# Nyro-Robotics/booster_gym

Measured on AMD Instinct MI355X. Metric: env-steps/sec (whole node), PPO rollout+update, T1 4096 envs/GPU, higher is better.
Workload: dtype f32

## Files before the change

booster_gym_amd/csrc/bg_env.h:

```cpp
#pragma once
#include "../../include/booster_gym_amd.h"
#include "bg_dyn.h"
#include "bg_rng.h"

namespace bg {

enum {
    F_ROOT = 0,
    F_Q = 13,
    F_QD = 25,
    F_LAST_TGT = 37,
    F_ACT = 49,
    F_LAST_ACT = 61,
    F_LAST_QD = 73,
    F_LAST_ROOTVEL = 85,
    F_CMD = 91,
    F_GAIT_F = 94,
    F_GAIT_P = 95,
    F_FILT_LIN = 96,
    F_FILT_ANG = 99,
    F_LAST_FEET = 102,
    F_PUSH = 108,
    F_CONTACT = 114,
    F_KP = 120, F_KD = 132, F_FRIC = 144,
// ... 77 lines not shown
    if (K <= 1u) return 0u;
    uint32_t bits = 2u;
    while (bits < 32u && (1u << bits) < K) bits += 2u;
    const uint32_t hb = bits >> 1, hm = (1u << hb) - 1u;
    uint32_t x = p;
    for (int walk = 0; walk < 64; walk++) {
        uint32_t L = x >> hb, R = x & hm;
        for (uint32_t r = 0; r < 4u; r++) {
            const uint32_t f = mix32(R ^ (key + r * 0x9E3779B9u)) & hm;
            const uint32_t t = L ^ f;
            L = R; R = t;
        }
        x = (L << hb) | R;
        if (x < K) return x;
    }
    return p;
}

template <int I, class St>
BG_HD void leg_fk(const St& st, const LegParams& lp, const LegState& ls, M3 Rpar, V3 ppar, M3* Rf, V3* pf) {
    constexpr int AX = LEG_AXIS[I], J = Plane<AX>::J, K = Plane<AX>::K;
    float s, c;
    bg_sincos(ls.q[I], &s, &c);
    V3 p = ppar + mul(Rpar, st.template link_pos<I>(lp));
    M3 R = Rpar;
    for (int r = 0; r < 3; r++) {
        R.e[r][J] = c * Rpar.e[r][J] + s * Rpar.e[r][K];
        R.e[r][K] = -s * Rpar.e[r][J] + c * Rpar.e[r][K];
    }
    if constexpr (I + 1 < LEG_LINKS) leg_fk<I + 1>(st, lp, ls, R, p, Rf, pf);
    else { *Rf = R; *pf = p; }
}

BG_HD Phys make_phys(const bg_env_cfg& c) {
    Phys ph;
    ph.dt = c.sim_dt; ph.g = v3(c.gravity[0], c.gravity[1], c.gravity[2]);
    ph.contact_ramp = c.contact_ramp; ph.friction_visc = c.friction_visc; ph.limit_k = c.limit_k; ph.limit_d = c.limit_d; ph.clamp_qd = c.clamp_qd;
    ph.body_gate = c.body_gate_height; ph.body_kn = c.contact_k; ph.body_dn = c.contact_d * (1.0f - 0.5f * c.terrain_restitution);
    ph.body_mu = 0.5f * (1.0f + c.terrain_mu);
    ph.zmask = 0;
    ph.self_on = c.self_collisions; ph.self_k = c.self_k; ph.self_d = c.self_d; ph.self_mu = c.self_mu; ph.self_visc = c.self_visc;
    return ph;
}
BG_HD ContactCfg make_contact_cfg(const bg_env_cfg& c) {
    ContactCfg cc; cc.k = c.contact_k; cc.d = c.contact_d; cc.terrain_mu = c.terrain_mu; cc.terrain_restitution = c.terrain_restitution;
    return cc;
}

BG_HD float quat_yaw(const float q[4]) {
    float x = q[0], y = q[1], z = q[2], w = q[3];
    return atan2f(2.f * (w * z + x * y), w * w + x * x - y * y - z * z);
}

struct GlobalSink {
    static constexpr int SELF = SELF_INLINE;
    float* obs; float* priv; int e;
    BG_HD void put_obs(int k, float v) { obs[(size_t)e * BG_NUM_OBS + k] = v; }
    BG_HD void put_priv(int k, float v) { priv[(size_t)e * BG_NUM_PRIV + k] = v; }
};

template <bool H16>
struct FieldRef {
    float* pf;
    bg_half_bits* ph;
    BG_HD operator float() const {
        if constexpr (H16) { if (ph) return half_bits_to_float(*ph); }
        return *pf;
    }
    BG_HD void operator=(float v) const {
        if constexpr (H16) { if (ph) { *ph = float_to_half_bits(v); return; } }
        *pf = v;
    }
};
template <bool H16>
BG_HD FieldRef<H16> field_ref(float* F, bg_half_bits* H, int idx, int n, int e) {
    const size_t o = (size_t)idx * n + e;
    return FieldRef<H16>{F + o, (H16 && fp16_state_field(idx)) ? H + o : nullptr};
}

template <class X, class Sink, bool H16, bool BODY, bool TC = false>
BG_HD void env_step_lane(const EnvDev& E, X& x, Sink& sink, int e, int leg, bool valid, const float* act, uint32_t step, int mode,
                         const StepOut& out) {
    const bg_env_cfg& C = E.cfg;
    const int n = E.n;
    const ModelDev& M = *E.model;
    float* const F = E.f;
    bg_half_bits* const HS = E.h;
    int32_t* const II = E.i;
#define FLD(off, comp) field_ref<H16>(F, HS, (off) + (comp), n, e)
    const int j0 = leg * LEG_LINKS;
    const float dt_env = C.sim_dt * (float)C.decimation;
    Phys ph = make_phys(C);
    ph.zmask = E.zmask;
    ContactCfg cc = make_contact_cfg(C);

    BaseState bs;
    for (int a = 0; a < 3; a++) { bs.pos.e[a] = FLD(F_ROOT, a); bs.vlin.e[a] = FLD(F_ROOT, 7 + a); bs.vang.e[a] = FLD(F_ROOT, 10 + a); }
    for (int a = 0; a < 4; a++) bs.quat[a] = FLD(F_ROOT, 3 + a);
    LegState ls;
    float last_tgt[LEG_LINKS], kp[LEG_LINKS], kd[LEG_LINKS], fric[LEG_LINKS], a6[LEG_LINKS], last_act[LEG_LINKS], last_qd[LEG_LINKS];
    for (int i = 0; i < LEG_LINKS; i++) {
        ls.q[i] = FLD(F_Q, j0 + i); ls.qd[i] = FLD(F_QD, j0 + i);
        last_tgt[i] = FLD(F_LAST_TGT, j0 + i);
        kp[i] = FLD(F_KP, j0 + i); kd[i] = FLD(F_KD, j0 + i); fric[i] = FLD(F_FRIC, j0 + i);
        last_act[i] = FLD(F_LAST_ACT, j0 + i); last_qd[i] = FLD(F_LAST_QD, j0 + i);
    }
    LegParams lp;
    load_leg_params(M, cc, leg, e, n, F + (size_t)F_MASS_SCALE * n, F + (size_t)F_COM_OFF * n, F + (size_t)F_FOOT_MAT * n, lp);
    LinkConst bk = load_base_link(M, e, n, F + (size_t)F_MASS_SCALE * n, F + (size_t)F_COM_OFF * n);
    int ep_len = II[(size_t)I_EP_LEN * n + e], cmd_time = II[(size_t)I_CMD_TIME * n + e], delay = II[(size_t)I_DELAY * n + e];
    float cmd[3] = {FLD(F_CMD, 0), FLD(F_CMD, 1), FLD(F_CMD, 2)};
    float gait_f = FLD(F_GAIT_F, 0), gait_p = FLD(F_GAIT_P, 0);
    V3 filt_lin = v3(FLD(F_FILT_LIN, 0), FLD(F_FILT_LIN, 1), FLD(F_FILT_LIN, 2));
    V3 filt_ang = v3(FLD(F_FILT_ANG, 0), FLD(F_FILT_ANG, 1), FLD(F_FILT_ANG, 2));
    V3 push_f = v3(FLD(F_PUSH, 0), FLD(F_PUSH, 1), FLD(F_PUSH, 2)), push_t = v3(FLD(F_PUSH, 3), FLD(F_PUSH, 4), FLD(F_PUSH, 5));
    V3 last_foot = v3(FLD(F_LAST_FEET, 3 * leg), FLD(F_LAST_FEET, 3 * leg + 1), FLD(F_LAST_FEET, 3 * leg + 2));
    float last_rootvel[6];
    for (int a = 0; a < 6; a++) last_rootvel[a] = FLD(F_LAST_ROOTVEL, a);

    float tmean[LEG_LINKS];
    float body_pen = 0.f, body_term = 0.f;
    V3 foot_force = v3(0.f, 0.f, 0.f);
    for (int i = 0; i < LEG_LINKS; i++) { tmean[i] = 0.f; a6[i] = FLD(F_ACT, j0 + i); }

    typename Sink::Ctx cx;
    sink.bind(cx, lp);
    if (mode == 0) {
        float target[LEG_LINKS];
        for (int i = 0; i < LEG_LINKS; i++) {
            float a = act[(size_t)e * BG_NUM_DOFS + j0 + i];
            if (((float_bits(a) >> 23) & 0xFFu) == 0xFFu) a = 0.f;
            a = fminf(fmaxf(a, -C.clip_actions), C.clip_actions);
            a6[i] = a;
            target[i] = C.default_dof_pos[j0 + i] + C.action_scale * a;
        }
        SV wrench = local_wrench_at_com(bk, push_f, push_t);
        for (int s = 0; s < C.decimation; s++) {
            float tau[LEG_LINKS];
            for (int i = 0; i < LEG_LINKS; i++) {
                if (delay == s) last_tgt[i] = target[i];
                tau[i] = pd_torque(kp[i], kd[i], fric[i], M.tau_lim[j0 + i], last_tgt[i], ls.q[i], ls.qd[i]);
                tmean[i] += tau[i];
            }
            BodyContactOut bo;
            BaseContribution mine = substep_pre<BODY, Sink::SELF>(ph, E.terrain, M, leg, lp, ls, tau, bs, cx, x, (const SV*)nullptr, &bo);
            body_pen = 0.f; body_term = 0.f;
            if constexpr (BODY) {
                V3 tf = bo.trunk;
                for (int a = 0; a < 3; a++) tf.e[a] += x.swap(tf.e[a]);
                const float trunk_hit = (leg == 0 && dot(tf, tf) > 1.0f) ? 1.f : 0.f;
                body_pen = (C.penalized_body_mask & 1) ? trunk_hit : 0.f;
                body_term = (C.terminate_body_mask & 1) ? trunk_hit : 0.f;
                for (int i = 0; i < LEG_LINKS - 1; i++) {
                    const float hit = dot(bo.link[i], bo.link[i]) > 1.0f ? 1.f : 0.f;
                    const int bit = 1 << (1 + j0 + i);
                    if (C.penalized_body_mask & bit) body_pen += hit;
                    if (C.terminate_body_mask & bit) body_term += hit;
                }
            } else {
                const float hit = dot(bo.link[SELF_SHANK], bo.link[SELF_SHANK]) > 1.0f ? 1.f : 0.f;
                const int bit = 1 << (1 + j0 + SELF_SHANK);
                body_pen = (C.penalized_body_mask & bit) ? hit : 0.f;
                body_term = (C.terminate_body_mask & bit) ? hit : 0.f;
            }
            BaseContribution both;
            for (int k = 0; k < 6; k++) { both.I.A.e[k] = mine.I.A.e[k] + x.swap(mine.I.A.e[k]); both.I.M.e[k] = mine.I.M.e[k] + x.swap(mine.I.M.e[k]); }
            for (int r = 0; r < 3; r++) for (int c2 = 0; c2 < 3; c2++) both.I.H.e[r][c2] = mine.I.H.e[r][c2] + x.swap(mine.I.H.e[r][c2]);
            for (int k = 0; k < 3; k++) { both.p.a.e[k] = mine.p.a.e[k] + x.swap(mine.p.a.e[k]); both.p.l.e[k] = mine.p.l.e[k] + x.swap(mine.p.l.e[k]); }
            float qdd[LEG_LINKS];
            V3 lin_w, ang_w;
            SV wr = wrench;
            if (s != 0) wr = sv_zero();
            substep_solve(ph, bk, lp, ls, cx, both, wr, qdd, &lin_w, &ang_w, &foot_force);
            substep_integrate(ph, lp, ls, bs, qdd, lin_w, ang_w);
        }
        for (int i = 0; i < LEG_LINKS; i++) tmean[i] *= 1.0f / (float)C.decimation;
    }

    uint32_t expo = 0;
    {
        const float st[13] = {bs.pos.e[0], bs.pos.e[1], bs.pos.e[2], bs.quat[0], bs.quat[1], bs.quat[2], bs.quat[3],
                              bs.vlin.e[0], bs.vlin.e[1], bs.vlin.e[2], bs.vang.e[0], bs.vang.e[1], bs.vang.e[2]};
        for (int k = 0; k < 13; k++) expo |= (uint32_t)(((float_bits(st[k]) >> 23) & 0xFFu) >= 0xE6u);
        for (int i = 0; i < LEG_LINKS; i++) {
            expo |= (uint32_t)(((float_bits(ls.q[i]) >> 23) & 0xFFu) >= 0xE6u);
            expo |= (uint32_t)(((float_bits(ls.qd[i]) >> 23) & 0xFFu) >= 0xE6u);
        }
    }
    float bad = expo ? 1.f : 0.f;
    bad = (bad != 0.f || x.swap(bad) != 0.f) ? 1.f : 0.f;
    if (bad != 0.f) {
        bs.pos = v3(0.f, 0.f, 1.f); bs.quat[0] = bs.quat[1] = bs.quat[2] = 0.f; bs.quat[3] = 1.f;
        bs.vlin = v3(0.f, 0.f, 0.f); bs.vang = v3(0.f, 0.f, 0.f);
        for (int i = 0; i < LEG_LINKS; i++) { ls.q[i] = 0.f; ls.qd[i] = 0.f; tmean[i] = 0.f; }
        foot_force = v3(0.f, 0.f, 0.f);
    }
    M3 R0 = quat_to_mat(bs.quat);
    V3 base_lin = mulT(R0, bs.vlin), base_ang = mulT(R0, bs.vang);
    V3 proj_g = mulT(R0, v3(0.f, 0.f, -1.f));
    if (mode == 0) {
        filt_lin = C.filter_weight * base_lin + (1.0f - C.filter_weight) * filt_lin;
        filt_ang = C.filter_weight * base_ang + (1.0f - C.filter_weight) * filt_ang;
    }
    M3 Rf; V3 pf;
    leg_fk<0>(cx.w.st, lp, ls, R0, bs.pos, &Rf, &pf);
    float roll = atan2f(Rf.e[2][1], Rf.e[2][2]), yaw = atan2f(Rf.e[1][0], Rf.e[0][0]);
    float fcontact = 0.f;
    for (int k = 0; k < 4; k++) {
        V3 xw = pf + mul(Rf, lp.corner[k]);
        if (xw.e[2] - terrain_height(E.terrain, xw.e[0], xw.e[1]) < 0.01f) fcontact = 1.f;
    }
    float s_tau2 = 0.f, s_tired = 0.f, s_power = 0.f, s_qd2 = 0.f, s_acc = 0.f, s_arate = 0.f, s_poslim = 0.f, s_vellim = 0.f, s_taulim = 0.f;
    for (int i = 0; i < LEG_LINKS; i++) {
        float lim = M.tau_lim[j0 + i], lo = M.q_lo[j0 + i], hi = M.q_hi[j0 + i];
        s_tau2 += tmean[i] * tmean[i];
        float tr = tmean[i] / lim;
        s_tired += fminf(tr * tr, 1.0f);
        s_power += fmaxf(tmean[i] * ls.qd[i], 0.f);
        s_qd2 += ls.qd[i] * ls.qd[i];
        float acc = (last_qd[i] - ls.qd[i]) / dt_env;
        s_acc += acc * acc;
        float da = last_act[i] - a6[i];
        s_arate += da * da;
        float lower = lo + 0.5f * (1.f - C.soft_dof_pos_limit) * (hi - lo), upper = hi - 0.5f * (1.f - C.soft_dof_pos_limit) * (hi - lo);
        s_poslim += (ls.q[i] < lower || ls.q[i] > upper) ? 1.f : 0.f;
        s_vellim += fminf(fmaxf(fabsf(ls.qd[i]) - M.qd_max[j0 + i] * C.soft_dof_vel_limit, 0.f), 1.f);
        s_taulim += fmaxf(fabsf(tmean[i]) - lim * C.soft_torque_limit, 0.f);
    }
    V3 dfoot = (1.0f / dt_env) * (last_foot - pf);
    float slip_own = dot(dfoot, dfoot) * fcontact;
    float velz_own = dfoot.e[2] * dfoot.e[2];
    V3 pf_o = v3(x.swap(pf.e[0]), x.swap(pf.e[1]), x.swap(pf.e[2]));
    float roll_o = x.swap(roll), yaw_o = x.swap(yaw), fcontact_o = x.swap(fcontact);
    s_tau2 += x.swap(s_tau2); s_tired += x.swap(s_tired); s_power += x.swap(s_power); s_qd2 += x.swap(s_qd2); s_acc += x.swap(s_acc);
    s_arate += x.swap(s_arate); s_poslim += x.swap(s_poslim); s_vellim += x.swap(s_vellim); s_taulim += x.swap(s_taulim);
    float slip = slip_own + x.swap(slip_own), velz = velz_own + x.swap(velz_own);
    V3 foot_force_o = v3(x.swap(foot_force.e[0]), x.swap(foot_force.e[1]), x.swap(foot_force.e[2]));
    V3 pL = leg == 0 ? pf : pf_o, pR = leg == 0 ? pf_o : pf;
    float yawL = leg == 0 ? yaw : yaw_o, yawR = leg == 0 ? yaw_o : yaw, rollL = leg == 0 ? roll : roll_o, rollR = leg == 0 ? roll_o : roll;
    float conL = leg == 0 ? fcontact : fcontact_o, conR = leg == 0 ? fcontact_o : fcontact;

    uint8_t reset_flag = 0, tout_flag = 0;
    float rew_total = 0.f;
    float term[BG_NUM_REWARD_TERMS];
    for (int k = 0; k < BG_NUM_REWARD_TERMS; k++) term[k] = 0.f;
    const uint32_t cnt = step + 1;
    const uint32_t so = mode ? 64u : 0u;

    if (mode == 0) {
        ep_len += 1;
        gait_p = fmodf(gait_p + dt_env * gait_f, 1.0f);
        if (C.kick_interval > 0 && cnt % (uint32_t)C.kick_interval == 0) {
            Rand4 r0 = rand4(C.seed, (uint32_t)e, step, so + RS_KICK0), r1 = rand4(C.seed, (uint32_t)e, step, so + RS_KICK1);
            for (int a = 0; a < 3; a++) bs.vlin.e[a] = apply_rand(bs.vlin.e[a], C.kick_lin_vel, r0.u[a], r0.n[a]);
            bs.vang.e[0] = apply_rand(bs.vang.e[0], C.kick_ang_vel, r0.u[3], r0.n[3]);
            bs.vang.e[1] = apply_rand(bs.vang.e[1], C.kick_ang_vel, r1.u[0], r1.n[0]);
            bs.vang.e[2] = apply_rand(bs.vang.e[2], C.kick_ang_vel, r1.u[1], r1.n[1]);
        }
        if (C.push_interval > 0) {
            uint32_t ph_ = cnt % (uint32_t)C.push_interval;
            if (ph_ == 0) {
                Rand4 r0 = rand4(C.seed, (uint32_t)e, step, so + RS_PUSH0), r1 = rand4(C.seed, (uint32_t)e, step, so + RS_PUSH1);
                for (int a = 0; a < 3; a++) push_f.e[a] = apply_rand(0.f, C.push_force, r0.u[a], r0.n[a]);
                push_t.e[0] = apply_rand(0.f, C.push_torque, r0.u[3], r0.n[3]);
                push_t.e[1] = apply_rand(0.f, C.push_torque, r1.u[0], r1.n[0]);
                push_t.e[2] = apply_rand(0.f, C.push_torque, r1.u[1], r1.n[1]);
            } else if (ph_ == (uint32_t)C.push_duration) {
                push_f = v3(0.f, 0.f, 0.f); push_t = v3(0.f, 0.f, 0.f);
            }
        }
        float h_base = terrain_height(E.terrain, bs.pos.e[0], bs.pos.e[1]);
        float v2 = dot(bs.vlin, bs.vlin) + dot(bs.vang, bs.vang);
        bool to = ep_len > C.max_episode_length;
        {
            const float hit = dot(foot_force, foot_force) > 1.0f ? 1.f : 0.f;
            const int bit = 1 << (1 + j0 + LEG_LINKS - 1);
            if (C.penalized_body_mask & bit) body_pen += hit;
            if (C.terminate_body_mask & bit) body_term += hit;
        }
        body_pen += x.swap(body_pen);
        body_term += x.swap(body_term);
        bool rs = (body_term > 0.f) || (v2 > C.terminate_vel) || (bs.pos.e[2] - h_base < C.terminate_height) || to;
        to = to || (ep_len == cmd_time);
        if (bad != 0.f) rs = true;
        reset_flag = rs ? 1 : 0; tout_flag = to ? 1 : 0;
        float base_yaw = quat_yaw(bs.quat);
        float bh = bs.pos.e[2] - h_base - C.base_height_target;
        float ex = cmd[0] - filt_lin.e[0], ey = cmd[1] - filt_lin.e[1], ew = cmd[2] - filt_ang.e[2];
        float racc = 0.f;
        {
            float rv[6] = {bs.vlin.e[0], bs.vlin.e[1], bs.vlin.e[2], bs.vang.e[0], bs.vang.e[1], bs.vang.e[2]};
            for (int a = 0; a < 6; a++) { float d = (last_rootvel[a] - rv[a]) / dt_env; racc += d * d; }
        }
        float ydiff = wrap_pi(yawR - yawL);
        float ymean = 0.5f * (yawL + yawR) + (fabsf(yawR - yawL) > 3.14159265358979f ? 3.14159265358979f : 0.f);
        float ymerr = wrap_pi(base_yaw - ymean);
        float fdist = fabsf(cosf(base_yaw) * (pR.e[1] - pL.e[1]) - sinf(base_yaw) * (pR.e[0] - pL.e[0]));
        bool gait_on = gait_f > 1.0e-8f;
        bool lsw = (fabsf(gait_p - 0.25f) < 0.5f * C.swing_period) && gait_on, rsw = (fabsf(gait_p - 0.75f) < 0.5f * C.swing_period) && gait_on;
        term[BG_REW_SURVIVAL] = 1.0f;
        term[BG_REW_TRACKING_LIN_VEL_X] = expf(-ex * ex / C.tracking_sigma);
        term[BG_REW_TRACKING_LIN_VEL_Y] = expf(-ey * ey / C.tracking_sigma);
        term[BG_REW_TRACKING_ANG_VEL] = expf(-ew * ew / C.tracking_sigma);
        term[BG_REW_BASE_HEIGHT] = bh * bh;
        term[BG_REW_ORIENTATION] = proj_g.e[0] * proj_g.e[0] + proj_g.e[1] * proj_g.e[1];
        term[BG_REW_TORQUES] = s_tau2;
        term[BG_REW_TORQUE_TIREDNESS] = s_tired;
        term[BG_REW_POWER] = s_power;
        term[BG_REW_LIN_VEL_Z] = filt_lin.e[2] * filt_lin.e[2];
        term[BG_REW_ANG_VEL_XY] = base_ang.e[0] * base_ang.e[0] + base_ang.e[1] * base_ang.e[1];
        term[BG_REW_DOF_VEL] = s_qd2;
        term[BG_REW_DOF_ACC] = s_acc;
        term[BG_REW_ROOT_ACC] = racc;
        term[BG_REW_ACTION_RATE] = s_arate;
        term[BG_REW_DOF_POS_LIMITS] = s_poslim;
        term[BG_REW_DOF_VEL_LIMITS] = s_vellim;
        term[BG_REW_TORQUE_LIMITS] = s_taulim;
        term[BG_REW_COLLISION] = body_pen;
        term[BG_REW_FEET_SLIP] = slip * (ep_len > 1 ? 1.f : 0.f);
        term[BG_REW_FEET_VEL_Z] = velz;
        term[BG_REW_FEET_YAW_DIFF] = ydiff * ydiff;
        term[BG_REW_FEET_YAW_MEAN] = ymerr * ymerr;
        term[BG_REW_FEET_ROLL] = rollL * rollL + rollR * rollR;
        term[BG_REW_FEET_DISTANCE] = fminf(fmaxf(C.feet_distance_ref - fdist, 0.f), 0.1f);
        term[BG_REW_FEET_SWING] = ((lsw && conL == 0.f) ? 1.f : 0.f) + ((rsw && conR == 0.f) ? 1.f : 0.f);
        for (int k = 0; k < BG_NUM_REWARD_TERMS; k++) {
            term[k] = C.reward_scale[k] != 0.f ? term[k] * C.reward_scale[k] : 0.f;
            rew_total += term[k];
        }
        if (C.only_positive_rewards) rew_total = fmaxf(rew_total, 0.f);
        if (bad != 0.f) { rew_total = 0.f; for (int k = 0; k < BG_NUM_REWARD_TERMS; k++) term[k] = 0.f; }
    } else {
        reset_flag = 1;
    }

    V3 pf_store = pf;
    if (reset_flag && mode == 0 && C.curriculum && leg == 0 && valid && bad == 0.f) {
        const int nx = 2 * C.lin_vel_levels + 1, ny = 2 * C.ang_vel_levels + 1;
        bool success = (float)ep_len > ceilf((float)C.max_episode_length) * (1.0f - C.episode_length_toler);
        success = success && fabsf(filt_lin.e[0] - cmd[0]) < C.lin_vel_x_toler && fabsf(filt_lin.e[1] - cmd[1]) < C.lin_vel_y_toler &&
                  fabsf(filt_ang.e[2] - cmd[2]) < C.ang_vel_yaw_toler;
        if (success) {
            const int cx = II[(size_t)I_CURR_LIN * n + e] + C.lin_vel_levels, cy = II[(size_t)I_CURR_ANG * n + e] + C.ang_vel_levels;
            const float r = C.curriculum_update_rate;
#if defined(__HIP_DEVICE_COMPILE__)
#define BG_ACC(ix, iy) atomicAdd(&E.curr[(ix) * ny + (iy)], r)
#else
#define BG_ACC(ix, iy) (E.curr[(ix) * ny + (iy)] += r)
#endif
            BG_ACC(cx, cy);
            if (cx > 0) BG_ACC(cx - 1, cy);
            if (cx < nx - 1) BG_ACC(cx + 1, cy);
            if (cy > 0) BG_ACC(cx, cy - 1);
            if (cy < ny - 1) BG_ACC(cx, cy + 1);
#undef BG_ACC
        }
    }
    float org_x = 0.f, org_y = 0.f;
    if constexpr (TC) {
        org_x = FLD(F_ORIGIN, 0); org_y = FLD(F_ORIGIN, 1);
        if (reset_flag && mode == 0 && valid && bad == 0.f) {
            int32_t* const TL = E.tcur;
            const int lvl = TL[e], col = TL[(size_t)n + e];
            const float dx = bs.pos.e[0] - org_x, dy = bs.pos.e[1] - org_y;
            const float d = sqrtf(dx * dx + dy * dy);
            const bool up = d > 0.5f * C.terrain_tile_length;
            const bool down = !up && d < sqrtf(cmd[0] * cmd[0] + cmd[1] * cmd[1]) * C.terrain_down_time;
            int nl = lvl + (up ? 1 : 0) - (down ? 1 : 0);
            nl = nl < 0 ? 0 : nl;
            if (nl >= C.terrain_num_levels) {
                nl = (int)(rand4(C.seed, (uint32_t)e, step, RS_TLEVEL).u[0] * (float)C.terrain_num_levels);
                nl = nl < C.terrain_num_levels ? nl : C.terrain_num_levels - 1;
            }
            org_x = ((float)col + 0.5f) * C.terrain_tile_width;
            org_y = ((float)nl + 0.5f) * C.terrain_tile_length;
            if (leg == 0) {
                TL[e] = nl;
                FLD(F_ORIGIN, 0) = org_x; FLD(F_ORIGIN, 1) = org_y; FLD(F_ORIGIN, 2) = terrain_height(E.terrain, org_x, org_y);
                if (nl != lvl) {
#if defined(__HIP_DEVICE_COMPILE__)
                    atomicAdd(&TL[2 * (size_t)n], nl - lvl);
#else
                    TL[2 * (size_t)n] += nl - lvl;
#endif
                }
            }
        }
    }
    if (reset_flag) {
        uint32_t noise_env = C.shared_reset_noise ? 0xFFFFFFFFu : (uint32_t)e;
        Rand4 d0 = rand4(C.seed, noise_env, step, so + RS_RESETDOF + leg * 2), d1 = rand4(C.seed, noise_env, step, so + RS_RESETDOF + leg * 2 + 1);
        for (int i = 0; i < LEG_LINKS; i++) {
            float u = i < 4 ? d0.u[i] : d1.u[i - 4], nn = i < 4 ? d0.n[i] : d1.n[i - 4];
            ls.q[i] = apply_rand(C.default_dof_pos[j0 + i], C.init_dof_pos, u, nn);
            ls.qd[i] = 0.f;
            last_tgt[i] = ls.q[i];
        }
        Rand4 r0 = rand4(C.seed, (uint32_t)e, step, so + RS_RESET0), r1 = rand4(C.seed, (uint32_t)e, step, so + RS_RESET1);
        float px = apply_rand(C.base_init_state[0] + (TC ? org_x : (float)FLD(F_ORIGIN, 0)), C.init_base_pos_xy, r0.u[0], r0.n[0]);
        float py = apply_rand(C.base_init_state[1] + (TC ? org_y : (float)FLD(F_ORIGIN, 1)), C.init_base_pos_xy, r0.u[1], r0.n[1]);
        bs.pos = v3(px, py, C.base_init_state[2] + terrain_height(E.terrain, px, py));
        float yw = r0.u[2] * 6.28318530717959f, sy, cy;
        bg_sincos(0.5f * yw, &sy, &cy);
        bs.quat[0] = 0.f; bs.quat[1] = 0.f; bs.quat[2] = sy; bs.quat[3] = cy;
        bs.vlin = v3(apply_rand(0.f, C.init_base_lin_vel_xy, r1.u[0], r1.n[0]), apply_rand(0.f, C.init_base_lin_vel_xy, r1.u[1], r1.n[1]), C.base_init_state[9]);
        bs.vang = v3(C.base_init_state[10], C.base_init_state[11], C.base_init_state[12]);
        ep_len = 0; cmd_time = 0;
        filt_lin = v3(0.f, 0.f, 0.f); filt_ang = v3(0.f, 0.f, 0.f);
        int dl = (int)(r0.u[3] * (float)C.decimation);
        delay = dl < C.decimation ? dl : C.decimation - 1;
    }
    if (mode == 0 && C.terrain_type != 0) {
        float sx = 0.f, sy2 = 0.f;
        float wx = C.terrain_env_width + C.terrain_border, wy = C.terrain_env_length + C.terrain_border;
        if (bs.pos.e[0] < -0.75f * C.terrain_border) sx += wx;
        if (bs.pos.e[0] > C.terrain_env_width + 0.75f * C.terrain_border) sx -= wx;
        if (bs.pos.e[1] < -0.75f * C.terrain_border) sy2 += wy;
        if (bs.pos.e[1] > C.terrain_env_length + 0.75f * C.terrain_border) sy2 -= wy;
        bs.pos.e[0] += sx; bs.pos.e[1] += sy2;
        pf_store.e[0] += sx; pf_store.e[1] += sy2;
    }
    const bool defer_still = C.exact_still_count != 0, defer_curr = C.curriculum && C.same_step_curriculum != 0;
    int resampled = 0;
    if (ep_len == cmd_time) {
        resampled = 1;
        Rand4 c0 = rand4(C.seed, (uint32_t)e, step, so + RS_CMD0), c1 = rand4(C.seed, (uint32_t)e, step, so + RS_CMD1);
        if (C.curriculum && !defer_curr) {
            Rand4 cr = rand4(C.seed, (uint32_t)e, step, so + RS_CURR);
            int lin_level, ang_level;
            curriculum_draw(C, E.curr_read, cr, cmd, &lin_level, &ang_level);
            if (leg == 0 && valid) { II[(size_t)I_CURR_LIN * n + e] = lin_level; II[(size_t)I_CURR_ANG * n + e] = ang_level; }
        } else if (!C.curriculum) {
            cmd[0] = C.cmd_lin_vel_x[0] + (C.cmd_lin_vel_x[1] - C.cmd_lin_vel_x[0]) * c0.u[0];
            cmd[1] = C.cmd_lin_vel_y[0] + (C.cmd_lin_vel_y[1] - C.cmd_lin_vel_y[0]) * c0.u[1];
            cmd[2] = C.cmd_ang_vel_yaw[0] + (C.cmd_ang_vel_yaw[1] - C.cmd_ang_vel_yaw[0]) * c0.u[2];
        }
        gait_f = C.cmd_gait_frequency[0] + (C.cmd_gait_frequency[1] - C.cmd_gait_frequency[0]) * c0.u[3];
        if (!defer_still && !defer_curr && c1.u[0] < C.still_proportion) { cmd[0] = cmd[1] = cmd[2] = 0.f; gait_f = 0.f; }
        int span = C.resample_steps[1] - C.resample_steps[0];
        int add = C.resample_steps[0] + (span > 0 ? (int)(c1.u[1] * (float)span) : 0);
        if (span > 0 && add >= C.resample_steps[1]) add = C.resample_steps[1] - 1;
        cmd_time += add;
    }
    if ((defer_still || defer_curr) && leg == 0 && valid) II[(size_t)I_RESAMPLED * n + e] = resampled;
    {
        Rand4 o0 = rand4(C.seed, (uint32_t)e, step, so + RS_OBS0), o1 = rand4(C.seed, (uint32_t)e, step, so + RS_OBS1), o2 = rand4(C.seed, (uint32_t)e, step, so + RS_OBS2);
        Rand4 p0 = rand4(C.seed, (uint32_t)e, step, so + RS_DOFPOS + leg * 2), p1 = rand4(C.seed, (uint32_t)e, step, so + RS_DOFPOS + leg * 2 + 1);
        Rand4 v0 = rand4(C.seed, (uint32_t)e, step, so + RS_DOFVEL + leg * 2), v1 = rand4(C.seed, (uint32_t)e, step, so + RS_DOFVEL + leg * 2 + 1);
        if (valid) {
            if (leg == 0) {
                for (int a = 0; a < 3; a++) sink.put_obs(a, apply_rand(proj_g.e[a], C.noise_gravity, o0.u[a], o0.n[a]) * C.norm_gravity);
                sink.put_obs(3, apply_rand(base_ang.e[0], C.noise_ang_vel, o0.u[3], o0.n[3]) * C.norm_ang_vel);
                sink.put_obs(4, apply_rand(base_ang.e[1], C.noise_ang_vel, o1.u[0], o1.n[0]) * C.norm_ang_vel);
                sink.put_obs(5, apply_rand(base_ang.e[2], C.noise_ang_vel, o1.u[1], o1.n[1]) * C.norm_ang_vel);
                sink.put_obs(6, cmd[0] * C.norm_lin_vel); sink.put_obs(7, cmd[1] * C.norm_lin_vel); sink.put_obs(8, cmd[2] * C.norm_ang_vel);
                float sg, cg;
                bg_sincos(6.28318530717959f * gait_p, &sg, &cg);
                float on = gait_f > 1.0e-8f ? 1.f : 0.f;
                sink.put_obs(9, cg * on); sink.put_obs(10, sg * on);
                for (int a = 0; a < 4; a++) sink.put_priv(a, FLD(F_BMS, a));
                sink.put_priv(4, apply_rand(base_lin.e[0], C.noise_lin_vel, o1.u[2], o1.n[2]) * C.norm_lin_vel);
                sink.put_priv(5, apply_rand(base_lin.e[1], C.noise_lin_vel, o1.u[3], o1.n[3]) * C.norm_lin_vel);
                sink.put_priv(6, apply_rand(base_lin.e[2], C.noise_lin_vel, o2.u[0], o2.n[0]) * C.norm_lin_vel);
                float hh = bs.pos.e[2] - terrain_height(E.terrain, bs.pos.e[0], bs.pos.e[1]);
                sink.put_priv(7, apply_rand(hh, C.noise_height, o2.u[1], o2.n[1]));
                for (int a = 0; a < 3; a++) { sink.put_priv(8 + a, push_f.e[a] * C.norm_push_force); sink.put_priv(11 + a, push_t.e[a] * C.norm_push_torque); }
            }
            for (int i = 0; i < LEG_LINKS; i++) {
                float up = i < 4 ? p0.u[i] : p1.u[i - 4], np_ = i < 4 ? p0.n[i] : p1.n[i - 4];
                float uv = i < 4 ? v0.u[i] : v1.u[i - 4], nv = i < 4 ? v0.n[i] : v1.n[i - 4];
                sink.put_obs(11 + j0 + i, apply_rand(ls.q[i] - C.default_dof_pos[j0 + i], C.noise_dof_pos, up, np_) * C.norm_dof_pos);
                sink.put_obs(23 + j0 + i, apply_rand(ls.qd[i], C.noise_dof_vel, uv, nv) * C.norm_dof_vel);
                sink.put_obs(35 + j0 + i, a6[i]);
            }
        }
    }
    if (!valid) return;
    for (int i = 0; i < LEG_LINKS; i++) {
        FLD(F_Q, j0 + i) = ls.q[i]; FLD(F_QD, j0 + i) = ls.qd[i];
        FLD(F_LAST_TGT, j0 + i) = last_tgt[i];
        FLD(F_ACT, j0 + i) = a6[i];
        if (mode == 0) { FLD(F_LAST_ACT, j0 + i) = a6[i]; FLD(F_TORQUES, j0 + i) = tmean[i]; }
        FLD(F_LAST_QD, j0 + i) = ls.qd[i];
    }
    for (int a = 0; a < 3; a++) {
        FLD(F_LAST_FEET, 3 * leg + a) = pf_store.e[a];
        FLD(F_FEET_POS, 3 * leg + a) = pf_store.e[a];
        FLD(F_CONTACT, 3 * leg + a) = foot_force.e[a];
    }
    FLD(F_FEET_ROLL, leg) = roll; FLD(F_FEET_YAW, leg) = yaw; FLD(F_FEET_CONTACT, leg) = fcontact;
    (void)foot_force_o;
    if (leg == 0) {
        for (int a = 0; a < 3; a++) {
            FLD(F_ROOT, a) = bs.pos.e[a]; FLD(F_ROOT, 7 + a) = bs.vlin.e[a]; FLD(F_ROOT, 10 + a) = bs.vang.e[a];
            FLD(F_LAST_ROOTVEL, a) = bs.vlin.e[a]; FLD(F_LAST_ROOTVEL, 3 + a) = bs.vang.e[a];
            FLD(F_CMD, a) = cmd[a];
            FLD(F_FILT_LIN, a) = filt_lin.e[a]; FLD(F_FILT_ANG, a) = filt_ang.e[a];
            FLD(F_PUSH, a) = push_f.e[a]; FLD(F_PUSH, 3 + a) = push_t.e[a];
            FLD(F_BASE_LIN, a) = base_lin.e[a]; FLD(F_BASE_ANG, a) = base_ang.e[a]; FLD(F_PROJ_G, a) = proj_g.e[a];
        }
        for (int a = 0; a < 4; a++) FLD(F_ROOT, 3 + a) = bs.quat[a];
        FLD(F_GAIT_F, 0) = gait_f; FLD(F_GAIT_P, 0) = gait_p;
        II[(size_t)I_EP_LEN * n + e] = ep_len; II[(size_t)I_CMD_TIME * n + e] = cmd_time; II[(size_t)I_DELAY * n + e] = delay;
        if (mode == 0) {
            out.rew[e] = rew_total; out.done[e] = reset_flag; out.tout[e] = tout_flag;
            if (out.terms) for (int k = 0; k < BG_NUM_REWARD_TERMS; k++) out.terms[(size_t)k * n + e] = term[k];
            int eps = II[(size_t)I_EP_STEPS * n + e] + 1;
            float es = FLD(F_EP_SUMS, 0) + rew_total;
            if (bad != 0.f) {
#if defined(__HIP_DEVICE_COMPILE__)
                atomicAdd(&E.stats[3 + BG_NUM_REWARD_TERMS], 1.0f);
#else
                E.stats[3 + BG_NUM_REWARD_TERMS] += 1.0f;
#endif
            }
            if (reset_flag) {
#if defined(__HIP_DEVICE_COMPILE__)
                atomicAdd(&E.stats[0], 1.0f); atomicAdd(&E.stats[1], (float)eps); atomicAdd(&E.stats[2], es);
#else
                E.stats[0] += 1.0f; E.stats[1] += (float)eps; E.stats[2] += es;
#endif
                es = 0.f; eps = 0;
            }
            FLD(F_EP_SUMS, 0) = es;
            II[(size_t)I_EP_STEPS * n + e] = eps;
            for (int k = 0; k < BG_NUM_REWARD_TERMS; k++) {
                if (C.reward_scale[k] == 0.f) continue;
                float t = FLD(F_EP_SUMS, 1 + k) + term[k];
                if (reset_flag) {
#if defined(__HIP_DEVICE_COMPILE__)
                    atomicAdd(&E.stats[3 + k], t);
#else
                    E.stats[3 + k] += t;
#endif
                    t = 0.f;
                }
                FLD(F_EP_SUMS, 1 + k) = t;
            }
        }
    }
#undef FLD
}

}
```

booster_gym_amd/csrc/bg_sim.hip:

```cpp
#include <hip/hip_runtime.h>
#include <stdio.h>
#include <string.h>
#include <string>
#include <vector>

#include "bg_env.h"
#include "bg_dyn_pk.h"
#include "bg_model.h"

using namespace bg;

static int fail(int code, const std::string& msg) { return bg_set_error(code, msg.c_str()); }
#define HIP_OK(expr)                                                                                 \
    do {                                                                                             \
        hipError_t _e = (expr);                                                                      \
        if (_e != hipSuccess) return fail(-2, std::string(#expr) + ": " + hipGetErrorString(_e));    \
    } while (0)



struct bg_env {
    bg_env_cfg cfg;
    bg_model_desc model;
    int n;
    float* f = nullptr;
    bg_half_bits* h = nullptr;
    int* rs_counts = nullptr;
    unsigned* lowmask = nullptr;
    bool body_two_kernel = false;
    unsigned* fd_mask = nullptr;
    int* fd_list = nullptr;
    unsigned* fd_count = nullptr;
    int32_t* i = nullptr;
    float* stats = nullptr;
    float* curr = nullptr;
    float* curr_read = nullptr;
    int curr_cells = 0;
    int32_t* tcur = nullptr;
    float* scan_xy = nullptr;
    float* hist = nullptr;
    int hist_head = 0;
    int hist_planes = 0;
    float* student_bound = nullptr;
    ModelDev* model_dev = nullptr;
    PairModel* pair_dev = nullptr;
    int16_t* hf = nullptr;
    TerrainDev terrain;
    StepOut bound;
    int64_t step_count = 0;
    int zmask = 0;
    int num_cus = 256;
    float *sim_root = nullptr, *sim_dof = nullptr, *sim_contact = nullptr, *sim_body = nullptr;
    float *sim_tau = nullptr, *sim_bforce = nullptr, *sim_btorque = nullptr;
    bool sim_wrench_pending = false;
};

struct DppSwap {
    __device__ __forceinline__ float swap(float v) {
        int r = __builtin_amdgcn_update_dpp(0, __float_as_int(v), 0xB1, 0xF, 0xF, true);
        return __int_as_float(r);
    }
};

struct LdsSink {
    static constexpr int SELF = SELF_INLINE;
    float* obs; float* priv; int el;
    lds_f32* self_sc; int lane;
    using Ctx = SubstepCtx;
    __device__ __forceinline__ void bind(Ctx& cx, const LegParams&) const { cx.w.self_sc = self_sc; cx.w.self_lane = lane; }
    __device__ __forceinline__ void put_obs(int k, float v) { obs[el * BG_NUM_OBS + k] = v; }
    __device__ __forceinline__ void put_priv(int k, float v) { priv[el * BG_NUM_PRIV + k] = v; }
};

constexpr int ENVS_PER_BLOCK = 32;
constexpr int BODY_GRID = 512;

__device__ __forceinline__ void copy_out_rows(const StepOut& out, int e0, int rows, unsigned mask, const float* s_obs, const float* s_priv) {
    const int lane = threadIdx.x;
    for (int r = 0; r < rows; r++) {
        if (!((mask >> r) & 1u)) continue;
        if (lane < BG_NUM_OBS) out.obs[(size_t)(e0 + r) * BG_NUM_OBS + lane] = s_obs[r * BG_NUM_OBS + lane];
        if (lane < BG_NUM_PRIV) out.priv[(size_t)(e0 + r) * out.priv_stride + lane] = s_priv[r * BG_NUM_PRIV + lane];
    }
}

template <bool H16, bool GATED, bool TC = false>
__global__ __launch_bounds__(64) void env_step_kernel(EnvDev E, const float* __restrict__ act, uint32_t step, int mode, StepOut out,
                                                      unsigned* __restrict__ lowmask) {
    __shared__ float s_obs[ENVS_PER_BLOCK * BG_NUM_OBS];
    __shared__ float s_priv[ENVS_PER_BLOCK * BG_NUM_PRIV];
    __shared__ float s_self[SELF_LDS_FLOATS];
    __shared__ unsigned s_low;
    const int lane = threadIdx.x;
    const int e0 = blockIdx.x * ENVS_PER_BLOCK;
    int e = e0 + (lane >> 1);
    const bool valid = e < E.n;
    if (!valid) e = E.n - 1;
    if (lane == 0) s_low = 0u;
    __syncthreads();
    DppSwap x;
    LdsSink sink{s_obs, s_priv, lane >> 1, (lds_f32*)s_self, lane};
    const V3 p0 = v3(E.f[(size_t)(F_ROOT + 0) * E.n + e], E.f[(size_t)(F_ROOT + 1) * E.n + e], E.f[(size_t)(F_ROOT + 2) * E.n + e]);
    const bool low = GATED && mode == 0 && body_contacts_active(make_phys(E.cfg), E.terrain, *E.model, p0);
    if (low) { if (valid && !(lane & 1)) atomicOr(&s_low, 1u << (lane >> 1)); }
    else env_step_lane<DppSwap, LdsSink, H16, false, TC>(E, x, sink, e, lane & 1, valid, act, step, mode, out);
    __syncthreads();
    const int rows = min(ENVS_PER_BLOCK, E.n - e0);
    const unsigned lowm = s_low;
    if (lowm == 0u) {
        float* go = out.obs + (size_t)e0 * BG_NUM_OBS;
        for (int k = lane; k < rows * BG_NUM_OBS; k += 64) go[k] = s_obs[k];
        float* gp = out.priv + (size_t)e0 * out.priv_stride;
        for (int k = lane; k < rows * BG_NUM_PRIV; k += 64) {
            const int r = k / BG_NUM_PRIV;
            gp[(size_t)r * out.priv_stride + (k - r * BG_NUM_PRIV)] = s_priv[k];
        }
    } else {
        copy_out_rows(out, e0, rows, ~lowm, s_obs, s_priv);
    }
    if (GATED && lane == 0) lowmask[blockIdx.x] = lowm;
}

template <bool H16, bool TC = false>
__global__ __launch_bounds__(64) void env_step_body_kernel(EnvDev E, const float* __restrict__ act, uint32_t step, StepOut out,
                                                           const unsigned* __restrict__ lowmask, int nblocks) {
    __shared__ float s_obs[ENVS_PER_BLOCK * BG_NUM_OBS];
    __shared__ float s_priv[ENVS_PER_BLOCK * BG_NUM_PRIV];
    __shared__ float s_self[SELF_LDS_FLOATS];
    const int lane = threadIdx.x;
    for (int b = blockIdx.x; b < nblocks; b += gridDim.x) {
        const unsigned lowm = lowmask[b];
        if (lowm == 0u) continue;
        const int e0 = b * ENVS_PER_BLOCK;
        int e = e0 + (lane >> 1);
        const bool valid = e < E.n;
        if (!valid) e = E.n - 1;
        DppSwap x;
        LdsSink sink{s_obs, s_priv, lane >> 1, (lds_f32*)s_self, lane};
        if ((lowm >> (lane >> 1)) & 1u) env_step_lane<DppSwap, LdsSink, H16, true, TC>(E, x, sink, e, lane & 1, valid, act, step, 0, out);
        __syncthreads();
        copy_out_rows(out, e0, min(ENVS_PER_BLOCK, E.n - e0), lowm, s_obs, s_priv);
        __syncthreads();
    }
}

constexpr int SCAN_BLOCK = 256;
template <bool H16>
__global__ __launch_bounds__(SCAN_BLOCK) void bg_height_scan(EnvDev E, const float2* __restrict__ pts, int P, float* __restrict__ priv, int stride) {
    const unsigned t = blockIdx.x * SCAN_BLOCK + threadIdx.x;
    if (t >= (unsigned)E.n * (unsigned)P) return;
    const int e = (int)(t / (unsigned)P), p = (int)(t - (unsigned)e * (unsigned)P);
    const int n = E.n;
#define SFLD(off) field_ref<H16>(E.f, E.h, (off), n, e)
    const float bx = SFLD(F_ROOT + 0), by = SFLD(F_ROOT + 1), bz = SFLD(F_ROOT + 2);
    const float q[4] = {SFLD(F_ROOT + 3), SFLD(F_ROOT + 4), SFLD(F_ROOT + 5), SFLD(F_ROOT + 6)};
#undef SFLD
    float s, c;
    bg_sincos(quat_yaw(q), &s, &c);
    const float2 pt = pts[p];
    const float h = terrain_height(E.terrain, bx + c * pt.x - s * pt.y, by + s * pt.x + c * pt.y);
    const float v = fminf(fmaxf(bz - h - E.cfg.base_height_target, -1.f), 1.f);
    priv[(size_t)e * stride + BG_NUM_PRIV + p] = v * E.cfg.height_scan_scale;
}

constexpr int PX_ENVS = 64, PX_BLOCK = 256, PX_MAX = 24, PX_LD = PX_MAX + 1;
static int priv_extras_columns(int mask) {
    return ((mask & BG_PRIV_EXTRA_FEET) ? 6 : 0) + ((mask & BG_PRIV_EXTRA_GROUND) ? 6 : 0) + ((mask & BG_PRIV_EXTRA_JOINTS) ? 12 : 0);
}
template <bool H16>
__global__ __launch_bounds__(PX_BLOCK) void bg_priv_extras(EnvDev E, float* __restrict__ priv, int stride, int off) {
    __shared__ float s_x[PX_ENVS * PX_LD];
    const int n = E.n, e0 = blockIdx.x * PX_ENVS, rows = min(PX_ENVS, n - e0);
    const int mask = E.cfg.priv_extras;
    const int c_ground = (mask & BG_PRIV_EXTRA_FEET) ? 6 : 0, c_joints = c_ground + ((mask & BG_PRIV_EXTRA_GROUND) ? 6 : 0);
    const int X = c_joints + ((mask & BG_PRIV_EXTRA_JOINTS) ? 12 : 0);
    const int role = threadIdx.x >> 6, el = threadIdx.x & 63, e = e0 + el;
    if (el < rows) {
        float* sx = s_x + el * PX_LD;
#define SFLD(off_) field_ref<H16>(E.f, E.h, (off_), n, e)
        if (role < 2) {
            if (mask & BG_PRIV_EXTRA_FEET) {
                const int leg = role;
                const float fz = SFLD(F_CONTACT + 3 * leg + 2);
                const float px = SFLD(F_FEET_POS + 3 * leg + 0), py = SFLD(F_FEET_POS + 3 * leg + 1), pz = SFLD(F_FEET_POS + 3 * leg + 2);
                sx[leg] = SFLD(F_FEET_CONTACT + leg);
                sx[2 + leg] = fminf(fmaxf(fz * E.cfg.priv_force_scale, -5.f), 5.f);
                sx[4 + leg] = fminf(fmaxf(pz - terrain_height(E.terrain, px, py), -1.f), 1.f) * E.cfg.priv_clearance_scale;
            }
        } else if (role == 2) {
            if (mask & BG_PRIV_EXTRA_GROUND) {
#pragma unroll
// ... 1154 lines not shown
```

Before: 4.654 million.

## Prefetch post-physics state into LDS park slots before substep loop

Measured after the change: 4.671 million (median of 6 runs). About the same (+0.4%).

```diff
diff --git a/booster_gym_amd/csrc/bg_env.h b/booster_gym_amd/csrc/bg_env.h
--- a/booster_gym_amd/csrc/bg_env.h
+++ b/booster_gym_amd/csrc/bg_env.h
@@ -153,11 +153,35 @@
     return atan2f(2.f * (w * z + x * y), w * w + x * x - y * y - z * z);
 }
 
+enum {
+    P_LAST_ACT = 0,
+    P_LAST_QD = 6,
+    P_ACT = 12,
+    P_Q_LO = 18, P_Q_HI = 24, P_QD_MAX = 30,
+    P_CMD = 36,
+    P_GAIT = 39,
+    P_FILT = 41,
+    P_PUSH = 47,
+    P_LAST_FOOT = 53,
+    P_LAST_ROOTVEL = 56,
+    P_BMS = 62,
+    P_ORIGIN = 66,
+    P_EP_SUMS = 68,
+    P_EP_LEN = 95, P_CMD_TIME = 96, P_EP_STEPS = 97,
+    PARK_SLOTS = 98
+};
+BG_HD float int_as_float(int32_t v) { float f; __builtin_memcpy(&f, &v, 4); return f; }
+BG_HD int32_t float_as_int(float f) { int32_t v; __builtin_memcpy(&v, &f, 4); return v; }
+
 struct GlobalSink {
     static constexpr int SELF = SELF_INLINE;
     float* obs; float* priv; int e;
+    float parked[PARK_SLOTS];
     BG_HD void put_obs(int k, float v) { obs[(size_t)e * BG_NUM_OBS + k] = v; }
     BG_HD void put_priv(int k, float v) { priv[(size_t)e * BG_NUM_PRIV + k] = v; }
+    BG_HD void park(int k, float v) { parked[k] = v; }
+    BG_HD float unpark(int k) const { return parked[k]; }
+    BG_HD void park_done() const {}
 };
 
 template <bool H16>
@@ -199,25 +223,35 @@
     for (int a = 0; a < 3; a++) { bs.pos.e[a] = FLD(F_ROOT, a); bs.vlin.e[a] = FLD(F_ROOT, 7 + a); bs.vang.e[a] = FLD(F_ROOT, 10 + a); }
     for (int a = 0; a < 4; a++) bs.quat[a] = FLD(F_ROOT, 3 + a);
     LegState ls;
-    float last_tgt[LEG_LINKS], kp[LEG_LINKS], kd[LEG_LINKS], fric[LEG_LINKS], a6[LEG_LINKS], last_act[LEG_LINKS], last_qd[LEG_LINKS];
+    float last_tgt[LEG_LINKS], kp[LEG_LINKS], kd[LEG_LINKS], fric[LEG_LINKS], tau_lim[LEG_LINKS], a6[LEG_LINKS];
     for (int i = 0; i < LEG_LINKS; i++) {
         ls.q[i] = FLD(F_Q, j0 + i); ls.qd[i] = FLD(F_QD, j0 + i);
         last_tgt[i] = FLD(F_LAST_TGT, j0 + i);
         kp[i] = FLD(F_KP, j0 + i); kd[i] = FLD(F_KD, j0 + i); fric[i] = FLD(F_FRIC, j0 + i);
-        last_act[i] = FLD(F_LAST_ACT, j0 + i); last_qd[i] = FLD(F_LAST_QD, j0 + i);
+        tau_lim[i] = M.tau_lim[j0 + i];
     }
     LegParams lp;
     load_leg_params(M, cc, leg, e, n, F + (size_t)F_MASS_SCALE * n, F + (size_t)F_COM_OFF * n, F + (size_t)F_FOOT_MAT * n, lp);
     LinkConst bk = load_base_link(M, e, n, F + (size_t)F_MASS_SCALE * n, F + (size_t)F_COM_OFF * n);
-    int ep_len = II[(size_t)I_EP_LEN * n + e], cmd_time = II[(size_t)I_CMD_TIME * n + e], delay = II[(size_t)I_DELAY * n + e];
-    float cmd[3] = {FLD(F_CMD, 0), FLD(F_CMD, 1), FLD(F_CMD, 2)};
-    float gait_f = FLD(F_GAIT_F, 0), gait_p = FLD(F_GAIT_P, 0);
-    V3 filt_lin = v3(FLD(F_FILT_LIN, 0), FLD(F_FILT_LIN, 1), FLD(F_FILT_LIN, 2));
-    V3 filt_ang = v3(FLD(F_FILT_ANG, 0), FLD(F_FILT_ANG, 1), FLD(F_FILT_ANG, 2));
+    int delay = II[(size_t)I_DELAY * n + e];
     V3 push_f = v3(FLD(F_PUSH, 0), FLD(F_PUSH, 1), FLD(F_PUSH, 2)), push_t = v3(FLD(F_PUSH, 3), FLD(F_PUSH, 4), FLD(F_PUSH, 5));
-    V3 last_foot = v3(FLD(F_LAST_FEET, 3 * leg), FLD(F_LAST_FEET, 3 * leg + 1), FLD(F_LAST_FEET, 3 * leg + 2));
-    float last_rootvel[6];
-    for (int a = 0; a < 6; a++) last_rootvel[a] = FLD(F_LAST_ROOTVEL, a);
+    for (int i = 0; i < LEG_LINKS; i++) {
+        sink.park(P_LAST_ACT + i, FLD(F_LAST_ACT, j0 + i)); sink.park(P_LAST_QD + i, FLD(F_LAST_QD, j0 + i));
+        sink.park(P_Q_LO + i, M.q_lo[j0 + i]); sink.park(P_Q_HI + i, M.q_hi[j0 + i]); sink.park(P_QD_MAX + i, M.qd_max[j0 + i]);
+    }
+    for (int a = 0; a < 3; a++) {
+        sink.park(P_CMD + a, FLD(F_CMD, a));
+        sink.park(P_FILT + a, FLD(F_FILT_LIN, a)); sink.park(P_FILT + 3 + a, FLD(F_FILT_ANG, a));
+        sink.park(P_PUSH + a, push_f.e[a]); sink.park(P_PUSH + 3 + a, push_t.e[a]);
+        sink.park(P_LAST_FOOT + a, FLD(F_LAST_FEET, 3 * leg + a));
+    }
+    sink.park(P_GAIT, FLD(F_GAIT_F, 0)); sink.park(P_GAIT + 1, FLD(F_GAIT_P, 0));
+    for (int a = 0; a < 6; a++) sink.park(P_LAST_ROOTVEL + a, FLD(F_LAST_ROOTVEL, a));
+    for (int a = 0; a < 4; a++) sink.park(P_BMS + a, FLD(F_BMS, a));
+    for (int a = 0; a < 2; a++) sink.park(P_ORIGIN + a, FLD(F_ORIGIN, a));
+    for (int k = 0; k < 1 + BG_NUM_REWARD_TERMS; k++) sink.park(P_EP_SUMS + k, FLD(F_EP_SUMS, k));
+    sink.park(P_EP_LEN, int_as_float(II[(size_t)I_EP_LEN * n + e])); sink.park(P_CMD_TIME, int_as_float(II[(size_t)I_CMD_TIME * n + e]));
+    sink.park(P_EP_STEPS, int_as_float(II[(size_t)I_EP_STEPS * n + e]));
 
     float tmean[LEG_LINKS];
     float body_pen = 0.f, body_term = 0.f;
@@ -226,8 +260,8 @@
 
     typename Sink::Ctx cx;
     sink.bind(cx, lp);
+    float target[LEG_LINKS];
     if (mode == 0) {
-        float target[LEG_LINKS];
         for (int i = 0; i < LEG_LINKS; i++) {
             float a = act[(size_t)e * BG_NUM_DOFS + j0 + i];
             if (((float_bits(a) >> 23) & 0xFFu) == 0xFFu) a = 0.f;
@@ -235,12 +269,15 @@
             a6[i] = a;
             target[i] = C.default_dof_pos[j0 + i] + C.action_scale * a;
         }
+    }
+    for (int i = 0; i < LEG_LINKS; i++) sink.park(P_ACT + i, a6[i]);
+    if (mode == 0) {
         SV wrench = local_wrench_at_com(bk, push_f, push_t);
         for (int s = 0; s < C.decimation; s++) {
             float tau[LEG_LINKS];
             for (int i = 0; i < LEG_LINKS; i++) {
                 if (delay == s) last_tgt[i] = target[i];
-                tau[i] = pd_torque(kp[i], kd[i], fric[i], M.tau_lim[j0 + i], last_tgt[i], ls.q[i], ls.qd[i]);
+                tau[i] = pd_torque(kp[i], kd[i], fric[i], tau_lim[i], last_tgt[i], ls.q[i], ls.qd[i]);
                 tmean[i] += tau[i];
             }
             BodyContactOut bo;
@@ -278,6 +315,23 @@
         for (int i = 0; i < LEG_LINKS; i++) tmean[i] *= 1.0f / (float)C.decimation;
     }
 
+    sink.park_done();
+    float last_act[LEG_LINKS], last_qd[LEG_LINKS], q_lo[LEG_LINKS], q_hi[LEG_LINKS], qd_max[LEG_LINKS];
+    for (int i = 0; i < LEG_LINKS; i++) {
+        last_act[i] = sink.unpark(P_LAST_ACT + i); last_qd[i] = sink.unpark(P_LAST_QD + i); a6[i] = sink.unpark(P_ACT + i);
+        q_lo[i] = sink.unpark(P_Q_LO + i); q_hi[i] = sink.unpark(P_Q_HI + i); qd_max[i] = sink.unpark(P_QD_MAX + i);
+    }
+    int ep_len = float_as_int(sink.unpark(P_EP_LEN)), cmd_time = float_as_int(sink.unpark(P_CMD_TIME));
+    float cmd[3] = {sink.unpark(P_CMD), sink.unpark(P_CMD + 1), sink.unpark(P_CMD + 2)};
+    float gait_f = sink.unpark(P_GAIT), gait_p = sink.unpark(P_GAIT + 1);
+    V3 filt_lin = v3(sink.unpark(P_FILT), sink.unpark(P_FILT + 1), sink.unpark(P_FILT + 2));
+    V3 filt_ang = v3(sink.unpark(P_FILT + 3), sink.unpark(P_FILT + 4), sink.unpark(P_FILT + 5));
+    push_f = v3(sink.unpark(P_PUSH), sink.unpark(P_PUSH + 1), sink.unpark(P_PUSH + 2));
+    push_t = v3(sink.unpark(P_PUSH + 3), sink.unpark(P_PUSH + 4), sink.unpark(P_PUSH + 5));
+    V3 last_foot = v3(sink.unpark(P_LAST_FOOT), sink.unpark(P_LAST_FOOT + 1), sink.unpark(P_LAST_FOOT + 2));
+    float last_rootvel[6];
+    for (int a = 0; a < 6; a++) last_rootvel[a] = sink.unpark(P_LAST_ROOTVEL + a);
+
     uint32_t expo = 0;
     {
         const float st[13] = {bs.pos.e[0], bs.pos.e[1], bs.pos.e[2], bs.quat[0], bs.quat[1], bs.quat[2], bs.quat[3],
@@ -313,7 +367,7 @@
     }
     float s_tau2 = 0.f, s_tired = 0.f, s_power = 0.f, s_qd2 = 0.f, s_acc = 0.f, s_arate = 0.f, s_poslim = 0.f, s_vellim = 0.f, s_taulim = 0.f;
     for (int i = 0; i < LEG_LINKS; i++) {
-        float lim = M.tau_lim[j0 + i], lo = M.q_lo[j0 + i], hi = M.q_hi[j0 + i];
+        float lim = tau_lim[i], lo = q_lo[i], hi = q_hi[i];
         s_tau2 += tmean[i] * tmean[i];
         float tr = tmean[i] / lim;
         s_tired += fminf(tr * tr, 1.0f);
@@ -325,7 +379,7 @@
         s_arate += da * da;
         float lower = lo + 0.5f * (1.f - C.soft_dof_pos_limit) * (hi - lo), upper = hi - 0.5f * (1.f - C.soft_dof_pos_limit) * (hi - lo);
         s_poslim += (ls.q[i] < lower || ls.q[i] > upper) ? 1.f : 0.f;
-        s_vellim += fminf(fmaxf(fabsf(ls.qd[i]) - M.qd_max[j0 + i] * C.soft_dof_vel_limit, 0.f), 1.f);
+        s_vellim += fminf(fmaxf(fabsf(ls.qd[i]) - qd_max[i] * C.soft_dof_vel_limit, 0.f), 1.f);
         s_taulim += fmaxf(fabsf(tmean[i]) - lim * C.soft_torque_limit, 0.f);
     }
     V3 dfoot = (1.0f / dt_env) * (last_foot - pf);
@@ -343,8 +397,8 @@
 
     uint8_t reset_flag = 0, tout_flag = 0;
     float rew_total = 0.f;
-    float term[BG_NUM_REWARD_TERMS];
-    for (int k = 0; k < BG_NUM_REWARD_TERMS; k++) term[k] = 0.f;
+    float term[BG_NUM_REWARD_TERMS], rscale[BG_NUM_REWARD_TERMS];
+    for (int k = 0; k < BG_NUM_REWARD_TERMS; k++) { term[k] = 0.f; rscale[k] = 0.f; }
     const uint32_t cnt = step + 1;
     const uint32_t so = mode ? 64u : 0u;
 
@@ -426,7 +480,8 @@
         term[BG_REW_FEET_DISTANCE] = fminf(fmaxf(C.feet_distance_ref - fdist, 0.f), 0.1f);
         term[BG_REW_FEET_SWING] = ((lsw && conL == 0.f) ? 1.f : 0.f) + ((rsw && conR == 0.f) ? 1.f : 0.f);
         for (int k = 0; k < BG_NUM_REWARD_TERMS; k++) {
-            term[k] = C.reward_scale[k] != 0.f ? term[k] * C.reward_scale[k] : 0.f;
+            rscale[k] = C.reward_scale[k];
+            term[k] = rscale[k] != 0.f ? term[k] * rscale[k] : 0.f;
             rew_total += term[k];
         }
         if (C.only_positive_rewards) rew_total = fmaxf(rew_total, 0.f);
@@ -459,7 +514,7 @@
     }
     float org_x = 0.f, org_y = 0.f;
     if constexpr (TC) {
-        org_x = FLD(F_ORIGIN, 0); org_y = FLD(F_ORIGIN, 1);
+        org_x = sink.unpark(P_ORIGIN); org_y = sink.unpark(P_ORIGIN + 1);
         if (reset_flag && mode == 0 && valid && bad == 0.f) {
             int32_t* const TL = E.tcur;
             const int lvl = TL[e], col = TL[(size_t)n + e];
@@ -498,8 +553,8 @@
             last_tgt[i] = ls.q[i];
         }
         Rand4 r0 = rand4(C.seed, (uint32_t)e, step, so + RS_RESET0), r1 = rand4(C.seed, (uint32_t)e, step, so + RS_RESET1);
-        float px = apply_rand(C.base_init_state[0] + (TC ? org_x : (float)FLD(F_ORIGIN, 0)), C.init_base_pos_xy, r0.u[0], r0.n[0]);
-        float py = apply_rand(C.base_init_state[1] + (TC ? org_y : (float)FLD(F_ORIGIN, 1)), C.init_base_pos_xy, r0.u[1], r0.n[1]);
+        float px = apply_rand(C.base_init_state[0] + (TC ? org_x : sink.unpark(P_ORIGIN)), C.init_base_pos_xy, r0.u[0], r0.n[0]);
+        float py = apply_rand(C.base_init_state[1] + (TC ? org_y : sink.unpark(P_ORIGIN + 1)), C.init_base_pos_xy, r0.u[1], r0.n[1]);
         bs.pos = v3(px, py, C.base_init_state[2] + terrain_height(E.terrain, px, py));
         float yw = r0.u[2] * 6.28318530717959f, sy, cy;
         bg_sincos(0.5f * yw, &sy, &cy);
@@ -559,7 +614,7 @@
                 bg_sincos(6.28318530717959f * gait_p, &sg, &cg);
                 float on = gait_f > 1.0e-8f ? 1.f : 0.f;
                 sink.put_obs(9, cg * on); sink.put_obs(10, sg * on);
-                for (int a = 0; a < 4; a++) sink.put_priv(a, FLD(F_BMS, a));
+                for (int a = 0; a < 4; a++) sink.put_priv(a, sink.unpark(P_BMS + a));
                 sink.put_priv(4, apply_rand(base_lin.e[0], C.noise_lin_vel, o1.u[2], o1.n[2]) * C.norm_lin_vel);
                 sink.put_priv(5, apply_rand(base_lin.e[1], C.noise_lin_vel, o1.u[3], o1.n[3]) * C.norm_lin_vel);
                 sink.put_priv(6, apply_rand(base_lin.e[2], C.noise_lin_vel, o2.u[0], o2.n[0]) * C.norm_lin_vel);
@@ -606,8 +661,10 @@
         if (mode == 0) {
             out.rew[e] = rew_total; out.done[e] = reset_flag; out.tout[e] = tout_flag;
             if (out.terms) for (int k = 0; k < BG_NUM_REWARD_TERMS; k++) out.terms[(size_t)k * n + e] = term[k];
-            int eps = II[(size_t)I_EP_STEPS * n + e] + 1;
-            float es = FLD(F_EP_SUMS, 0) + rew_total;
+            float ep_sum[1 + BG_NUM_REWARD_TERMS];
+            for (int k = 0; k < 1 + BG_NUM_REWARD_TERMS; k++) ep_sum[k] = sink.unpark(P_EP_SUMS + k);
+            int eps = float_as_int(sink.unpark(P_EP_STEPS)) + 1;
+            float es = ep_sum[0] + rew_total;
             if (bad != 0.f) {
 #if defined(__HIP_DEVICE_COMPILE__)
                 atomicAdd(&E.stats[3 + BG_NUM_REWARD_TERMS], 1.0f);
@@ -626,8 +683,8 @@
             FLD(F_EP_SUMS, 0) = es;
             II[(size_t)I_EP_STEPS * n + e] = eps;
             for (int k = 0; k < BG_NUM_REWARD_TERMS; k++) {
-                if (C.reward_scale[k] == 0.f) continue;
-                float t = FLD(F_EP_SUMS, 1 + k) + term[k];
+                if (rscale[k] == 0.f) continue;
+                float t = ep_sum[1 + k] + term[k];
                 if (reset_flag) {
 #if defined(__HIP_DEVICE_COMPILE__)
                     atomicAdd(&E.stats[3 + k], t);
diff --git a/booster_gym_amd/csrc/bg_sim.hip b/booster_gym_amd/csrc/bg_sim.hip
--- a/booster_gym_amd/csrc/bg_sim.hip
+++ b/booster_gym_amd/csrc/bg_sim.hip
@@ -66,10 +66,14 @@
     static constexpr int SELF = SELF_INLINE;
     float* obs; float* priv; int el;
     lds_f32* self_sc; int lane;
+    float* park_lane;
     using Ctx = SubstepCtx;
     __device__ __forceinline__ void bind(Ctx& cx, const LegParams&) const { cx.w.self_sc = self_sc; cx.w.self_lane = lane; }
     __device__ __forceinline__ void put_obs(int k, float v) { obs[el * BG_NUM_OBS + k] = v; }
     __device__ __forceinline__ void put_priv(int k, float v) { priv[el * BG_NUM_PRIV + k] = v; }
+    __device__ __forceinline__ void park(int k, float v) { park_lane[k * 64] = v; }
+    __device__ __forceinline__ float unpark(int k) const { return park_lane[k * 64]; }
+    __device__ __forceinline__ void park_done() const { asm volatile("" ::: "memory"); }
 };
 
 constexpr int ENVS_PER_BLOCK = 32;
@@ -90,6 +94,7 @@
     __shared__ float s_obs[ENVS_PER_BLOCK * BG_NUM_OBS];
     __shared__ float s_priv[ENVS_PER_BLOCK * BG_NUM_PRIV];
     __shared__ float s_self[SELF_LDS_FLOATS];
+    __shared__ float s_park[PARK_SLOTS * 64];
     __shared__ unsigned s_low;
     const int lane = threadIdx.x;
     const int e0 = blockIdx.x * ENVS_PER_BLOCK;
@@ -99,7 +104,7 @@
     if (lane == 0) s_low = 0u;
     __syncthreads();
     DppSwap x;
-    LdsSink sink{s_obs, s_priv, lane >> 1, (lds_f32*)s_self, lane};
+    LdsSink sink{s_obs, s_priv, lane >> 1, (lds_f32*)s_self, lane, s_park + lane};
     const V3 p0 = v3(E.f[(size_t)(F_ROOT + 0) * E.n + e], E.f[(size_t)(F_ROOT + 1) * E.n + e], E.f[(size_t)(F_ROOT + 2) * E.n + e]);
     const bool low = GATED && mode == 0 && body_contacts_active(make_phys(E.cfg), E.terrain, *E.model, p0);
     if (low) { if (valid && !(lane & 1)) atomicOr(&s_low, 1u << (lane >> 1)); }
@@ -127,6 +132,7 @@
     __shared__ float s_obs[ENVS_PER_BLOCK * BG_NUM_OBS];
     __shared__ float s_priv[ENVS_PER_BLOCK * BG_NUM_PRIV];
     __shared__ float s_self[SELF_LDS_FLOATS];
+    __shared__ float s_park[PARK_SLOTS * 64];
     const int lane = threadIdx.x;
     for (int b = blockIdx.x; b < nblocks; b += gridDim.x) {
         const unsigned lowm = lowmask[b];
@@ -136,7 +142,7 @@
         const bool valid = e < E.n;
         if (!valid) e = E.n - 1;
         DppSwap x;
-        LdsSink sink{s_obs, s_priv, lane >> 1, (lds_f32*)s_self, lane};
+        LdsSink sink{s_obs, s_priv, lane >> 1, (lds_f32*)s_self, lane, s_park + lane};
         if ((lowm >> (lane >> 1)) & 1u) env_step_lane<DppSwap, LdsSink, H16, true, TC>(E, x, sink, e, lane & 1, valid, act, step, 0, out);
         __syncthreads();
         copy_out_rows(out, e0, min(ENVS_PER_BLOCK, E.n - e0), lowm, s_obs, s_priv);
```
